# google/deepconsensus

Measured on NVIDIA H100. Metric: zmw_windows_per_sec, higher is better.
Workload: dtype bf16

## Files before the change

deepconsensus_b200/csrc/engine.cu:

```cuda
#include <cuda_bf16.h>
#include <cuda_runtime.h>
#include <math.h>
#include <stdarg.h>
#include <stdio.h>
#include <string.h>

#include <algorithm>
#include <cmath>
#include <functional>
#include <map>
#include <memory>
#include <string>
#include <vector>

#include "../../include/dcb200.h"
#include "../../include/dcb200_debug.h"
#include "kernels.h"

using namespace dcb;

namespace {

thread_local std::string g_create_error;

// ... 556 lines not shown
  epi.x = e->d_x;
  epi.bias = bias;
  if (pos && c.add_pos_encoding) { epi.pe = e->w.pe; epi.pe_img = e->w.pe_img; }
  if (layer < c.num_hidden_layers) {
    epi.xb = e->d_xb;
    if (!c.rezero) { epi.ln_g = e->w.layers[layer].ln_g[sub]; epi.ln_b = e->w.layers[layer].ln_b[sub]; }
  }
  epi.has_xold = has_xold;
  epi.L = e->Lw;
  return epi;
}

struct DbgImage { int stage, which; const DevBuf<__nv_bfloat16>* src; int width; };

std::vector<DbgImage> dbg_images(const dcb_engine* e) {
  const int layers = e->cfg.num_hidden_layers, ff = e->cfg.filter_size;
  std::vector<DbgImage> v = {{0, DCB_DEBUG_EMBED, &e->d_embqkv, e->Epad}, {0, DCB_DEBUG_XB, &e->d_xb, kDP}};
  for (int n = 0; n < layers; ++n) {
    v.insert(v.end(), {{1 + 2 * n, DCB_DEBUG_QKV, &e->d_embqkv, kQKVN}, {1 + 2 * n, DCB_DEBUG_ATT, &e->d_att, kDP},
                       {1 + 2 * n, DCB_DEBUG_XB, &e->d_xb, kDP}, {2 + 2 * n, DCB_DEBUG_HID, &e->d_hid, ff}});
    if (n + 1 < layers) v.push_back({2 + 2 * n, DCB_DEBUG_XB, &e->d_xb, kDP});
  }
  return v;
}

bool dbg_operand_slot(const dcb_engine* e, int stage, int which, size_t* cols, int* width) {
  *cols = 0;
  for (const DbgImage& im : dbg_images(e)) {
    if (im.stage == stage && im.which == which) { *width = im.width; return true; }
    *cols += im.width;
  }
  return false;
}

template <int K, typename T>
int read_capture(dcb_engine* e, const T* image, int iw, int ow, T* out, int64_t out_elems) {
  const int Mlay = e->last_chunk_tokens;
  const int M = Mlay / e->Lw * e->L;
  if (out_elems < (int64_t)M * ow) return fail(e, DCB_ERR_INVALID, "output too small: need %lld", (long long)M * ow);
  CU(e, cudaSetDevice(e->cfg.device));
  std::vector<T> img((size_t)(Mlay + kTileM - 1) / kTileM * kTileM * iw);
  CU(e, cudaMemcpy(img.data(), image, img.size() * sizeof(T), cudaMemcpyDeviceToHost));
  for (int t = 0; t < M; ++t) {
    const int tl = t / e->L * e->Lw + t % e->L;
    const int tile = tl / kTileM, r = tl % kTileM;
    for (int col = 0; col < ow; ++col)
      out[(size_t)t * ow + col] = img[(((size_t)tile * (iw / K) + col / K) * kTileM + r) * K + col % K];
  }
  return DCB_OK;
}

void bf16_forward_chunk(dcb_engine* e, LaunchRecorder& rec, const float* rows_chunk, const uint8_t* packed_chunk,
                        int bw, HeadParams hp, int* d_status) {
  const dcb_config& c = e->cfg;
  const Weights& W = e->w;
  const int L = e->L, Lw = e->Lw, M = bw * Lw;
  const int T = (M + kTileM - 1) / kTileM;
  const cudaStream_t st = rec.st;
  int stage = 0;
  auto snap = [&]() {
    if (e->debug) {
      const size_t ximg = x_image_elems(), cw = (size_t)e->chunk_tiles * kTileM;
      cudaMemcpyAsync(e->d_dbg + (size_t)stage * e->chunk_tiles * ximg, e->d_x, T * ximg * sizeof(float), cudaMemcpyDeviceToDevice, st);
      size_t cols = 0;
      for (const DbgImage& im : dbg_images(e)) {
        if (im.stage == stage)
          cudaMemcpyAsync(e->d_dbg_op + cols * cw, im.src->p, (size_t)T * kTileM * im.width * sizeof(__nv_bfloat16),
                          cudaMemcpyDeviceToDevice, st);
        cols += im.width;
      }
    }
    ++stage;
  };
  rec.run(kProfEmbed, 1, [&] {
    launch_embed(rows_chunk, packed_chunk, e->pl, e->R, L, Lw, M, T, e->echunks, W.cols, W.rowmeta, W.tables,
                 e->table_elems, e->d_embqkv, d_status, st);
  });
  rec.run(kProfRowGemm, 1, [&] {
    launch_gemm_row(e->d_embqkv, W.wc, e->Epad / 16, 2 * (e->Epad / 16), T, row_epi(e, false, nullptr, 0, 0, true), st);
  });
  snap();
  for (int n_ = 0; n_ < c.num_hidden_layers; ++n_) {
    const LayerDev& ld = W.layers[n_];
    rec.run(kProfQkv, 1, [&] { launch_gemm_qkv(e->d_xb, ld.wqkv, T, e->d_embqkv, st); });
    rec.run(kProfAttention, 1, [&] { launch_attention(e->d_embqkv, e->d_att, L, Lw, c.attn_win_size, bw, st); });
    rec.run(kProfRowGemm, 1, [&] {
      launch_gemm_row(e->d_att, ld.wo, kDP / 16, 2 * (kDP / 16), T, row_epi(e, true, nullptr, n_, 1, false), st);
    });
    snap();
    rec.run(kProfFfn, 2, [&] {
      const RowEpi epi = row_epi(e, true, ld.b2, n_ + 1, 0, false);
      __nv_bfloat16* hid = e->debug ? e->d_hid.p : nullptr;
      for (int half = 0; half < 2; ++half) launch_ffn(half, e->d_xb, ld.w1, ld.b1, ld.w2, c.filter_size, T, hid, epi, st);
    });
    if (e->profile) e->prof_ffn_tokens += (long long)bw * L;
    snap();
  }
  hp.x = e->d_x; hp.M = M; hp.L = L; hp.Lw = Lw;
  rec.run(kProfHead, 1, [&] { launch_head(hp, T, st); });
  e->last_chunk_tokens = M;
}

}

extern "C" {

const char* dcb_version(void) { return "dcb200 0.1.0 (sm_90a)"; }

const char* dcb_last_error(const dcb_engine* e) { return e ? e->err.c_str() : g_create_error.c_str(); }

int dcb_create(const dcb_config* cfg, dcb_engine** out) {
  if (!cfg || !out) return fail(nullptr, DCB_ERR_INVALID, "null argument");
  if (cfg->struct_size != (int32_t)sizeof(dcb_config))
    return fail(nullptr, DCB_ERR_INVALID, "dcb_config size mismatch: got %d, built with %zu",
                cfg->struct_size, sizeof(dcb_config));
  if (cfg->hidden_size != kD || cfg->num_heads != kHeads)
    return fail(nullptr, DCB_ERR_INVALID, "unsupported model: hidden_size=%d num_heads=%d (engine is built for %d/%d)",
                cfg->hidden_size, cfg->num_heads, kD, kHeads);
  if (!cfg->condense_transformer_input)
    return fail(nullptr, DCB_ERR_INVALID, "condense_transformer_input must be true");
  if (cfg->filter_size <= 0 || cfg->filter_size % kFFChunk || cfg->filter_size > 2048)
    return fail(nullptr, DCB_ERR_INVALID, "filter_size must be a multiple of %d and <= 2048", kFFChunk);
  if (cfg->max_passes <= 0 || cfg->max_length <= 0 || cfg->max_length > 256 || cfg->num_hidden_layers <= 0 ||
      cfg->max_batch <= 0)
    return fail(nullptr, DCB_ERR_INVALID, "bad max_passes/max_length(<=256)/num_hidden_layers/max_batch");
  if (cfg->precision != DCB_PRECISION_BF16 && cfg->precision != DCB_PRECISION_FP32)
    return fail(nullptr, DCB_ERR_INVALID, "precision must be DCB_PRECISION_BF16 or DCB_PRECISION_FP32");
  int ndev = 0;
  if (cudaGetDeviceCount(&ndev) != cudaSuccess || ndev == 0)
    return fail(nullptr, DCB_ERR_CUDA, "no CUDA device available (the dcb200 engine has no CPU fallback)");
  if (cfg->device < 0 || cfg->device >= ndev) return fail(nullptr, DCB_ERR_INVALID, "bad device ordinal %d", cfg->device);
  cudaDeviceProp prop;
  if (cudaGetDeviceProperties(&prop, cfg->device) != cudaSuccess || prop.major != 9)
    return fail(nullptr, DCB_ERR_CUDA, "device %d is not an sm_90 GPU (compute capability %d.%d)", cfg->device,
                prop.major, prop.minor);

  std::unique_ptr<dcb_engine> eng(new dcb_engine());
  dcb_engine* e = eng.get();
  e->cfg = *cfg;
  e->num_sms = prop.multiProcessorCount;
  e->L = cfg->max_length;
  e->Lw = e->L;
  bool align = true;
#ifdef DCB_DEV_SWITCHES
  if (const char* env = getenv("DCB_ALIGN")) align = atoi(env) != 0;
#endif
  if (align && e->L <= kTileM) e->Lw = kTileM;
  e->R = 4 * cfg->max_passes + (cfg->use_ccs_bq ? 6 : 5);
  e->pl = make_packed_layout(cfg->max_passes, cfg->max_length, cfg->use_ccs_bq ? 1 : 0);
  {
    auto table = [&](const char* layer, int vocab, int width) {
      const int off = (e->table_elems + 7) / 8 * 8;
      e->tables.push_back(EmbedTable{layer, vocab, width, off});
      e->table_elems = off + vocab * width;
      return e->tables.back();
    };
    auto rows = [&](const EmbedTable& tb, int n, float clip, int shift) {
      for (int r = 0; r < n; ++r) {
        e->embed.push_back(StrictEmbedRow{clip, shift, tb.vocab, tb.width, e->E, tb.off});
        e->E += tb.width;
      }
    };
    const int P = cfg->max_passes;
    const EmbedTable bases = table("bases_embedding_layer", kVocab, cfg->per_base_hidden_size);
    rows(bases, P, 0.f, 0);
    rows(table("pw_embedding_layer", cfg->pw_max + 1, cfg->pw_hidden_size), P, (float)cfg->pw_max, 0);
    rows(table("ip_embedding_layer", cfg->ip_max + 1, cfg->ip_hidden_size), P, (float)cfg->ip_max, 0);
    rows(table("strand_embedding_layer", cfg->strand_max + 1, cfg->strand_hidden_size), P, 0.f, 0);
// ... 846 lines not shown
```

deepconsensus_b200/csrc/kernels.cu:

```cuda
#include "kernels.h"

#include <cuda_bf16.h>
#include <math.h>
#include <stdio.h>
#include <stdlib.h>

#include "head_finish.cuh"
#include "sm90.cuh"

namespace dcb {


__global__ void __launch_bounds__(256)
embed_rows_kernel(const float* __restrict__ rows, const uint8_t* __restrict__ packed, PackedLayout pl, int R, int L,
                  int Lw, int M, int echunks,
                  const EmbedCol* __restrict__ cols, const EmbedRow* __restrict__ rowmeta,
                  const __nv_bfloat16* __restrict__ tables, int table_elems,
                  __nv_bfloat16* __restrict__ emb, int* __restrict__ status) {
  extern __shared__ __align__(1024) uint8_t smem[];
  __nv_bfloat16* s_tab = reinterpret_cast<__nv_bfloat16*>(smem);
  const int tab_bytes = (table_elems * 2 + 15) & ~15;
  EmbedCol* s_cols = reinterpret_cast<EmbedCol*>(smem + tab_bytes);
  const int cols_bytes = (echunks * 8 * (int)sizeof(EmbedCol) + 15) & ~15;
  uint16_t* s_ids = reinterpret_cast<uint16_t*>(smem + tab_bytes + cols_bytes);
// ... 477 lines not shown
      wgmma_fence_regs(hacc);
      if (c + 1 == nch) mbar_arrive(a_empty);

      uint32_t af[Cfg::kDownK][4];
      const float* bc = reinterpret_cast<const float*>(stage_base + prev * Cfg::kStageBytes + Cfg::kB1Off) + 2 * q;
#pragma unroll
      for (int kk = 0; kk < Cfg::kDownK; ++kk)
#pragma unroll
        for (int i = 0; i < 4; ++i) {
          const float2 b = *reinterpret_cast<const float2*>(bc + 16 * kk + 8 * (i >> 1));
          af[kk][i] = pack_bf16x2(fmaxf(hacc[8 * kk + 2 * i] + b.x, 0.f), fmaxf(hacc[8 * kk + 2 * i + 1] + b.y, 0.f));
        }
      mbar_arrive(&empty[prev]);
      if constexpr (kHid) {
        __nv_bfloat16* hb = hid + (size_t)tile * kTileM * ff + (size_t)row0 * 8 + 2 * q;
#pragma unroll
        for (int kk = 0; kk < Cfg::kDownK; ++kk)
#pragma unroll
          for (int i = 0; i < 4; ++i)
            *reinterpret_cast<uint32_t*>(hb + ((size_t)(c * 16 + 2 * kk + (i >> 1)) * kTileM + 8 * (i & 1)) * 8) =
                af[kk][i];
      }

#pragma unroll
      for (int kk = 0; kk < Cfg::kDownK; ++kk) {
        mbar_wait(&full[slot], phase);
        const uint32_t st = smem_u32(stage_base + slot * Cfg::kStageBytes);
        wgmma_fence_regs(acc[0]);
        wgmma_fence_regs(acc[1]);
        wgmma_fence();
#pragma unroll
        for (int j = 0; j < 2; ++j)
          wgmma_m64n144k16_rs(acc[j], af[kk], make_kc16_desc(st + j * kNC * 16, kDP * 16, 128), c != 0 || kk != 0);
        wgmma_commit();
        wgmma_fence_regs(acc[0]);
        wgmma_fence_regs(acc[1]);
        wgmma_wait<1>();
        if (kk > 0) {
          wgmma_fence_regs(af[kk - 1]);
          mbar_arrive(&empty[prev]);
        }
        prev = slot;
        next_slot();
      }
      wgmma_wait<0>();
      wgmma_fence_regs(acc[0]);
      wgmma_fence_regs(acc[1]);
      wgmma_fence_regs(af[Cfg::kDownK - 1]);
      mbar_arrive(&empty[prev]);
    }

    row_epilogue<kNC, 2, false>(acc, tile, row0, q, s_vec, epi);
  }
}

constexpr int kAttStride = 144;
constexpr int kAttChunks = kDHP / 8;

__device__ __forceinline__ void mma_bf16_16816(float (&c)[4], const uint32_t (&a)[4], uint32_t b0,
                                               uint32_t b1) {
  asm volatile(
      "mma.sync.aligned.m16n8k16.row.col.f32.bf16.bf16.f32 {%0,%1,%2,%3}, {%4,%5,%6,%7}, {%8,%9}, "
      "{%0,%1,%2,%3};"
      : "+f"(c[0]), "+f"(c[1]), "+f"(c[2]), "+f"(c[3])
      : "r"(a[0]), "r"(a[1]), "r"(a[2]), "r"(a[3]), "r"(b0), "r"(b1));
}

__device__ __forceinline__ void ldmatrix_x2_trans(uint32_t& r0, uint32_t& r1, uint32_t addr) {
  asm volatile("ldmatrix.sync.aligned.m8n8.x2.trans.shared.b16 {%0, %1}, [%2];"
               : "=r"(r0), "=r"(r1)
               : "r"(addr));
}

__device__ __forceinline__ size_t img_off(int tok, int col, int chunks) {
  const int tile = tok / kTileM, r = tok % kTileM;
  return (((size_t)tile * chunks + (col >> 3)) * kTileM + r) * 8 + (col & 7);
}

__device__ __forceinline__ int att_rot(int chunk, int rowmod) {
  const int t = chunk + rowmod;
  return t >= kAttChunks ? t - kAttChunks : t;
}

__global__ void __launch_bounds__(128, 3)
band_attention_kernel(const __nv_bfloat16* __restrict__ qkv, __nv_bfloat16* __restrict__ att,
                      int L, int Lw, int win, int nwindows) {
  extern __shared__ __align__(1024) uint8_t smem[];
  const int w = blockIdx.x >> 1;
  const int head = blockIdx.x & 1;
  if (w >= nwindows) return;
  const int Lp = (L + 15) & ~15;
  __nv_bfloat16* sK = reinterpret_cast<__nv_bfloat16*>(smem);
  __nv_bfloat16* sV = sK + (size_t)Lp * kAttStride;
  constexpr int qkv_chunks = kQKVN / 8;
  const int kcol = (2 + head) * kDHP, vcol = (4 + head) * kDHP, qcol = head * kDHP;
  const int tok0 = w * Lw;

  for (int row = threadIdx.x; row < Lp; row += blockDim.x) {
    const int rm = row % kAttChunks;
    __nv_bfloat16* dk = sK + (size_t)row * kAttStride;
    __nv_bfloat16* dv = sV + (size_t)row * kAttStride;
    if (row < L) {
      const int tok = tok0 + row;
      const size_t base = ((size_t)(tok / kTileM) * qkv_chunks) * kTileM * 8 + (size_t)(tok % kTileM) * 8;
      const __nv_bfloat16* gk = qkv + base + (size_t)(kcol >> 3) * kTileM * 8;
      const __nv_bfloat16* gv = qkv + base + (size_t)(vcol >> 3) * kTileM * 8;
#pragma unroll
      for (int ch = 0; ch < kAttChunks; ++ch) {
        const int pc = att_rot(ch, rm) * 8;
        asm volatile("cp.async.cg.shared.global [%0], [%1], 16;" ::"r"(smem_u32(dk + pc)),
                     "l"(gk + (size_t)ch * kTileM * 8) : "memory");
        asm volatile("cp.async.cg.shared.global [%0], [%1], 16;" ::"r"(smem_u32(dv + pc)),
                     "l"(gv + (size_t)ch * kTileM * 8) : "memory");
      }
    } else {
#pragma unroll
      for (int ch = 0; ch < kAttChunks; ++ch) {
        *reinterpret_cast<uint4*>(dk + ch * 8) = make_uint4(0, 0, 0, 0);
        *reinterpret_cast<uint4*>(dv + ch * 8) = make_uint4(0, 0, 0, 0);
      }
    }
  }
  asm volatile("cp.async.commit_group;" ::: "memory");

  const int warp = threadIdx.x >> 5, lane = threadIdx.x & 31;
  const int g = lane >> 2, t = lane & 3;
  const int band = win > 0 ? win : L;
  constexpr float kLog2e = 1.4426950408889634f;

  constexpr int kChunkElems = kTileM * 8;
  uint32_t qa[kDHP / 16][4];
  auto load_q = [&](int qb) {
    const int r0 = qb * 16 + g, r1 = r0 + 8;
    const __nv_bfloat16* q0 = qkv + img_off(tok0 + (r0 < L ? r0 : 0), qcol + 2 * t, qkv_chunks);
    const __nv_bfloat16* q1 = qkv + img_off(tok0 + (r1 < L ? r1 : 0), qcol + 2 * t, qkv_chunks);
#pragma unroll
    for (int ks = 0; ks < kDHP / 16; ++ks) {
      const uint32_t v0 = __ldg(reinterpret_cast<const uint32_t*>(q0 + (2 * ks) * kChunkElems));
      const uint32_t v1 = __ldg(reinterpret_cast<const uint32_t*>(q1 + (2 * ks) * kChunkElems));
      const uint32_t v2 = __ldg(reinterpret_cast<const uint32_t*>(q0 + (2 * ks + 1) * kChunkElems));
      const uint32_t v3 = __ldg(reinterpret_cast<const uint32_t*>(q1 + (2 * ks + 1) * kChunkElems));
      qa[ks][0] = r0 < L ? v0 : 0u;
      qa[ks][1] = r1 < L ? v1 : 0u;
      qa[ks][2] = r0 < L ? v2 : 0u;
      qa[ks][3] = r1 < L ? v3 : 0u;
    }
  };
  if (warp * 16 < L) load_q(warp);
  asm volatile("cp.async.wait_group 0;" ::: "memory");
  __syncthreads();

  for (int qb = warp; qb * 16 < L; qb += 4) {
    const int i0 = qb * 16;
    const int r0 = i0 + g, r1 = i0 + g + 8;
    if (qb != warp) load_q(qb);
    float o[kDHP / 8][4];
#pragma unroll
    for (int nt = 0; nt < kDHP / 8; ++nt) { o[nt][0] = o[nt][1] = o[nt][2] = o[nt][3] = 0.f; }
    float m0 = -INFINITY, m1 = -INFINITY, l0 = 0.f, l1 = 0.f;

    int jlo = i0 - band; if (jlo < 0) jlo = 0; jlo &= ~15;
    int jhi = i0 + 15 + band + 1; if (jhi > L) jhi = L;
    for (int j0 = jlo; j0 < jhi; j0 += 16) {
      float s[2][4], s2[2][4];
#pragma unroll
      for (int nt = 0; nt < 2; ++nt) {
        s[nt][0] = s[nt][1] = s[nt][2] = s[nt][3] = 0.f;
        s2[nt][0] = s2[nt][1] = s2[nt][2] = s2[nt][3] = 0.f;
      }
      const int krow0 = j0 + g, krow1 = j0 + 8 + g;
      const __nv_bfloat16* kr0 = sK + (size_t)krow0 * kAttStride + 2 * t;
      const __nv_bfloat16* kr1 = sK + (size_t)krow1 * kAttStride + 2 * t;
      const int km0 = krow0 % kAttChunks, km1 = krow1 % kAttChunks;
#pragma unroll
      for (int ks = 0; ks < kDHP / 16; ++ks) {
        const uint32_t a0 = *reinterpret_cast<const uint32_t*>(kr0 + att_rot(2 * ks, km0) * 8);
        const uint32_t a1 = *reinterpret_cast<const uint32_t*>(kr0 + att_rot(2 * ks + 1, km0) * 8);
        const uint32_t c0 = *reinterpret_cast<const uint32_t*>(kr1 + att_rot(2 * ks, km1) * 8);
        const uint32_t c1 = *reinterpret_cast<const uint32_t*>(kr1 + att_rot(2 * ks + 1, km1) * 8);
        if (ks & 1) {
          mma_bf16_16816(s2[0], qa[ks], a0, a1);
          mma_bf16_16816(s2[1], qa[ks], c0, c1);
        } else {
          mma_bf16_16816(s[0], qa[ks], a0, a1);
          mma_bf16_16816(s[1], qa[ks], c0, c1);
        }
      }
#pragma unroll
      for (int nt = 0; nt < 2; ++nt)
#pragma unroll
        for (int e = 0; e < 4; ++e) s[nt][e] += s2[nt][e];
      float tmax0 = -INFINITY, tmax1 = -INFINITY;
#pragma unroll
      for (int nt = 0; nt < 2; ++nt) {
#pragma unroll
        for (int e = 0; e < 4; ++e) {
          const int i = (e < 2) ? r0 : r1;
          const int j = j0 + nt * 8 + 2 * t + (e & 1);
          const int dlt = i - j;
          const bool ok = (j < L) && (dlt <= band) && (dlt >= -band);
          s[nt][e] = ok ? s[nt][e] : -INFINITY;
        }
        tmax0 = fmaxf(tmax0, fmaxf(s[nt][0], s[nt][1]));
        tmax1 = fmaxf(tmax1, fmaxf(s[nt][2], s[nt][3]));
      }
      tmax0 = fmaxf(tmax0, __shfl_xor_sync(0xffffffffu, tmax0, 1));
      tmax0 = fmaxf(tmax0, __shfl_xor_sync(0xffffffffu, tmax0, 2));
      tmax1 = fmaxf(tmax1, __shfl_xor_sync(0xffffffffu, tmax1, 1));
      tmax1 = fmaxf(tmax1, __shfl_xor_sync(0xffffffffu, tmax1, 2));
      const float mn0 = fmaxf(m0, tmax0), mn1 = fmaxf(m1, tmax1);
      const float base0 = mn0 == -INFINITY ? 0.f : mn0, base1 = mn1 == -INFINITY ? 0.f : mn1;
      const float sc0 = exp2f((m0 - base0) * kLog2e), sc1 = exp2f((m1 - base1) * kLog2e);
      m0 = mn0; m1 = mn1;
      float ps0 = 0.f, ps1 = 0.f;
      uint32_t pa[4];
      {
        float p[2][4];
#pragma unroll
        for (int nt = 0; nt < 2; ++nt) {
          p[nt][0] = exp2f((s[nt][0] - base0) * kLog2e);
          p[nt][1] = exp2f((s[nt][1] - base0) * kLog2e);
          p[nt][2] = exp2f((s[nt][2] - base1) * kLog2e);
          p[nt][3] = exp2f((s[nt][3] - base1) * kLog2e);
          ps0 += p[nt][0] + p[nt][1];
          ps1 += p[nt][2] + p[nt][3];
        }
        pa[0] = pack_bf16x2(p[0][0], p[0][1]);
        pa[1] = pack_bf16x2(p[0][2], p[0][3]);
        pa[2] = pack_bf16x2(p[1][0], p[1][1]);
        pa[3] = pack_bf16x2(p[1][2], p[1][3]);
      }
      l0 = l0 * sc0 + ps0;
      l1 = l1 * sc1 + ps1;
      const int vrow = j0 + (lane & 15);
      const int vm = vrow % kAttChunks;
      const uint32_t vbase = smem_u32(sV + (size_t)vrow * kAttStride);
#pragma unroll
      for (int nt = 0; nt < kDHP / 8; ++nt) {
        o[nt][0] *= sc0; o[nt][1] *= sc0; o[nt][2] *= sc1; o[nt][3] *= sc1;
        uint32_t b0, b1;
        ldmatrix_x2_trans(b0, b1, vbase + att_rot(nt, vm) * 16);
        mma_bf16_16816(o[nt], pa, b0, b1);
      }
    }
    l0 += __shfl_xor_sync(0xffffffffu, l0, 1);
    l0 += __shfl_xor_sync(0xffffffffu, l0, 2);
    l1 += __shfl_xor_sync(0xffffffffu, l1, 1);
    l1 += __shfl_xor_sync(0xffffffffu, l1, 2);
    const float inv0 = 1.f / l0, inv1 = 1.f / l1;
    __nv_bfloat16* o0 = att + img_off(tok0 + (r0 < L ? r0 : 0), head * kDHP + 2 * t, kDP / 8);
    __nv_bfloat16* o1 = att + img_off(tok0 + (r1 < L ? r1 : 0), head * kDHP + 2 * t, kDP / 8);
#pragma unroll
    for (int nt = 0; nt < kDHP / 8; ++nt) {
      if (r0 < L)
        *reinterpret_cast<uint32_t*>(o0 + nt * kChunkElems) = pack_bf16x2(o[nt][0] * inv0, o[nt][1] * inv0);
      if (r1 < L)
        *reinterpret_cast<uint32_t*>(o1 + nt * kChunkElems) = pack_bf16x2(o[nt][2] * inv1, o[nt][3] * inv1);
    }
  }
}

__global__ void __launch_bounds__(128)
head_kernel(HeadParams p) {
  __shared__ __align__(16) float sGW[kD * 8];
  __shared__ float sA[kVocab], sBj[kVocab];
  for (int i = threadIdx.x; i < kD * 2; i += blockDim.x)
    reinterpret_cast<float4*>(sGW)[i] = __ldg(reinterpret_cast<const float4*>(p.gw8) + i);
  if (threadIdx.x < kVocab) { sA[threadIdx.x] = p.ab[threadIdx.x]; sBj[threadIdx.x] = p.ab[8 + threadIdx.x]; }
  __syncthreads();
  const int tile = blockIdx.x, r = threadIdx.x;
  const int tok = tile * kTileM + r;
  if (tok >= p.M) return;
  const int wdw = tok / p.Lw, pos = tok - wdw * p.Lw;
  if (pos >= p.L) return;
  const size_t oidx = (size_t)wdw * p.L + pos;
  const float4* xrow = reinterpret_cast<const float4*>(p.x + (size_t)tile * x_image_elems()) + r;
  float s1 = 0.f, s2 = 0.f;
  float t[kVocab];
#pragma unroll
  for (int j = 0; j < kVocab; ++j) t[j] = 0.f;
  const float shift = xrow[0].x;
  constexpr int kHB = 10;
  static_assert((kD / 4) % kHB == 0, "head batch");
#pragma unroll 1
  for (int c0 = 0; c0 < kD / 4; c0 += kHB) {
    float4 v[kHB];
#pragma unroll
    for (int u = 0; u < kHB; ++u) v[u] = xrow[(size_t)(c0 + u) * kTileM];
#pragma unroll
    for (int u = 0; u < kHB; ++u) {
      const float ys[4] = {v[u].x - shift, v[u].y - shift, v[u].z - shift, v[u].w - shift};
#pragma unroll
      for (int i = 0; i < 4; ++i) {
        const int col = (c0 + u) * 4 + i;
        s1 += ys[i];
        s2 = fmaf(ys[i], ys[i], s2);
        const float4 w0 = *reinterpret_cast<const float4*>(&sGW[col * 8]);
        const float w4 = sGW[col * 8 + 4];
        t[0] = fmaf(ys[i], w0.x, t[0]); t[1] = fmaf(ys[i], w0.y, t[1]); t[2] = fmaf(ys[i], w0.z, t[2]);
        t[3] = fmaf(ys[i], w0.w, t[3]); t[4] = fmaf(ys[i], w4, t[4]);
      }
    }
  }
  const float m1 = s1 * (1.f / kD);
  const float rstd = rsqrtf(fmaxf(s2 * (1.f / kD) - m1 * m1, 0.f) + 1e-6f);
  float lg[kVocab];
#pragma unroll
  for (int j = 0; j < kVocab; ++j) lg[j] = rstd * (t[j] - m1 * sA[j]) + sBj[j];
  head_finish(p, lg, oidx);
}

static int g_num_sms = 0;
static int num_sms() {
  if (!g_num_sms) {
    int dev = 0;
    cudaGetDevice(&dev);
    cudaDeviceGetAttribute(&g_num_sms, cudaDevAttrMultiProcessorCount, dev);
    if (g_num_sms <= 0) g_num_sms = 132;
  }
  return g_num_sms;
}


template <int BN, int NCH, int EPI, bool kAres>
static cudaError_t gemm_init() {
  return cudaFuncSetAttribute(gemm_kernel<BN, NCH, EPI, kAres>, cudaFuncAttributeMaxDynamicSharedMemorySize,
                              GemmCfg<BN, NCH, kAres>::kSmemBytes);
}

cudaError_t kernels_init() {
  cudaError_t e;
  if ((e = gemm_init<kNC, 2, EPI_ROW, false>()) != cudaSuccess) return e;
  if ((e = gemm_init<kNC, 1, EPI_QKV, true>()) != cudaSuccess) return e;
  for (auto fn : {ffn_gemm_kernel<false>, ffn_gemm_kernel<true>})
    if ((e = cudaFuncSetAttribute(fn, cudaFuncAttributeMaxDynamicSharedMemorySize, FfnCfg::kSmemBytes)) != cudaSuccess)
      return e;
  e = cudaFuncSetAttribute(embed_rows_kernel, cudaFuncAttributeMaxDynamicSharedMemorySize, 160 * 1024);
  if (e != cudaSuccess) return e;
  e = cudaFuncSetAttribute(band_attention_kernel, cudaFuncAttributeMaxDynamicSharedMemorySize,
                           2 * 256 * kAttStride * 2);
  return e;
}

size_t embed_smem_bytes(int R, int echunks, int table_elems) {
  return (size_t)((table_elems * 2 + 15) & ~15) + ((echunks * 8 * sizeof(EmbedCol) + 15) & ~(size_t)15) +
         (size_t)R * kTileM * 2;
}

void launch_embed(const float* rows, const uint8_t* packed, const PackedLayout& pl, int R, int L, int Lw, int M, int ntiles, int echunks,
                  const EmbedCol* cols, const EmbedRow* rowmeta, const __nv_bfloat16* tables,
                  int table_elems, __nv_bfloat16* emb, int* status, cudaStream_t st) {
  embed_rows_kernel<<<ntiles, 256, embed_smem_bytes(R, echunks, table_elems), st>>>(
      rows, packed, pl, R, L, Lw, M, echunks, cols, rowmeta, tables, table_elems, emb, status);
}

void launch_gemm_row(const __nv_bfloat16* a_img, const __nv_bfloat16* b_img, int a_ksteps, int b_ksteps, int ntiles,
                     const RowEpi& epi, cudaStream_t st) {
  using Cfg = GemmCfg<kNC, 2, false>;
  const int grid = ntiles < num_sms() ? ntiles : num_sms();
  const int smem = Cfg::smem_bytes(Cfg::stages(b_ksteps / Cfg::kSK));
  gemm_kernel<kNC, 2, EPI_ROW, false><<<grid, Cfg::kThreads, smem, st>>>(a_img, b_img, a_ksteps, b_ksteps, ntiles, 1,
                                                                                    nullptr, 0, epi);
}

void launch_gemm_qkv(const __nv_bfloat16* a_img, const __nv_bfloat16* b_img, int ntiles,
                     __nv_bfloat16* qkv_img, cudaStream_t st) {
  using Cfg = GemmCfg<kNC, 1, true>;
  const int npairs = (ntiles + 1) / 2;
  const int grid = npairs < num_sms() ? npairs : num_sms();
  RowEpi none{};
  gemm_kernel<kNC, 1, EPI_QKV, true><<<grid, Cfg::kThreads, Cfg::kSmemBytes, st>>>(
      a_img, b_img, kDP / 16, 2 * (kDP / 16), ntiles, kQKVN / kQKVGroup, qkv_img, kQKVN / 8, none);
}

void launch_ffn(int half, const __nv_bfloat16* xb_img, const __nv_bfloat16* w1_img, const float* b1,
                const __nv_bfloat16* w2_img, int ff, int ntiles, __nv_bfloat16* hid_img, const RowEpi& epi,
                cudaStream_t st) {
  const int split = (ntiles + 1) / 2;
  const int t0 = half ? split : 0, t1 = half ? ntiles : split;
  const int n = t1 - t0;
  const int grid = n < 1 ? 1 : n < num_sms() ? n : num_sms();
  if (hid_img)
    ffn_gemm_kernel<true><<<grid, FfnCfg::kThreads, FfnCfg::kSmemBytes, st>>>(xb_img, w1_img, b1, w2_img, ff, t0, t1,
                                                                              hid_img, epi);
  else
    ffn_gemm_kernel<false><<<grid, FfnCfg::kThreads, FfnCfg::kSmemBytes, st>>>(xb_img, w1_img, b1, w2_img, ff, t0, t1,
                                                                               nullptr, epi);
}

__global__ void __launch_bounds__(256)
unpack_rows_kernel(const uint8_t* __restrict__ packed, PackedLayout pl, int nwindows, float* __restrict__ rows) {
  const int b = blockIdx.x;
  const uint8_t* w = packed + (size_t)b * pl.stride;
  float* out = rows + (size_t)b * pl.R * pl.L;
  for (int i = threadIdx.x; i < pl.R * pl.L; i += blockDim.x) {
    const int r = i / pl.L, l = i - r * pl.L;
    out[i] = packed_value(pl, w, r, l);
  }
}

void launch_unpack_rows(const uint8_t* packed, const PackedLayout& pl, int nwindows, float* rows, cudaStream_t st) {
  if (nwindows > 0) unpack_rows_kernel<<<nwindows, 256, 0, st>>>(packed, pl, nwindows, rows);
}


void launch_attention(const __nv_bfloat16* qkv, __nv_bfloat16* att, int L, int Lw, int win, int nwindows,
                      cudaStream_t st) {
  const int Lp = (L + 15) & ~15;
  const size_t smem = (size_t)2 * Lp * kAttStride * 2;
  band_attention_kernel<<<nwindows * 2, 128, smem, st>>>(qkv, att, L, Lw, win, nwindows);
}



__global__ void __launch_bounds__(256)
stitch_kernel(const uint8_t* __restrict__ bases, const uint8_t* __restrict__ quals, int L,
              const int32_t* __restrict__ zmw_start, uint8_t* __restrict__ seq_out, uint8_t* __restrict__ qual_out,
              int32_t* __restrict__ len_out) {
  __shared__ int s_warp[8];
  __shared__ int s_total;
  const int z = blockIdx.x;
  const size_t off = (size_t)zmw_start[z] * L;
  const int n = (zmw_start[z + 1] - zmw_start[z]) * L;
  const uint8_t* in_b = bases + off;
  const uint8_t* in_q = quals + off;
  uint8_t* out_b = seq_out + off;
  uint8_t* out_q = qual_out + off;
  const int warp = threadIdx.x >> 5, lane = threadIdx.x & 31;
  int running = 0;
  for (int t0 = 0; t0 < n; t0 += 1024) {
    uint8_t b[4], q[4];
    int cnt = 0;
#pragma unroll
    for (int k = 0; k < 4; ++k) {
      const int idx = t0 + threadIdx.x * 4 + k;
      b[k] = idx < n ? in_b[idx] : (uint8_t)' ';
      q[k] = idx < n ? in_q[idx] : (uint8_t)0;
      cnt += b[k] != (uint8_t)' ';
    }
    int incl = cnt;
#pragma unroll
    for (int d = 1; d < 32; d <<= 1) {
      const int v = __shfl_up_sync(0xffffffffu, incl, d);
      if (lane >= d) incl += v;
    }
    if (lane == 31) s_warp[warp] = incl;
    __syncthreads();
    if (threadIdx.x == 0) {
      int acc = 0;
      for (int w = 0; w < 8; ++w) { const int v = s_warp[w]; s_warp[w] = acc; acc += v; }
      s_total = acc;
    }
    __syncthreads();
    int pos = running + s_warp[warp] + incl - cnt;
#pragma unroll
    for (int k = 0; k < 4; ++k) {
      if (b[k] != (uint8_t)' ') {
        out_b[pos] = b[k];
        out_q[pos] = q[k];
        ++pos;
      }
    }
    running += s_total;
    __syncthreads();
  }
  if (threadIdx.x == 0) len_out[z] = running;
}

void launch_stitch(const uint8_t* bases, const uint8_t* quals, int L, const int32_t* zmw_start, int n_zmw,
                   uint8_t* seq_out, uint8_t* qual_out, int32_t* len_out, cudaStream_t st) {
  if (n_zmw > 0) stitch_kernel<<<n_zmw, 256, 0, st>>>(bases, quals, L, zmw_start, seq_out, qual_out, len_out);
}

void launch_head(const HeadParams& p, int ntiles, cudaStream_t st) {
  head_kernel<<<ntiles, 128, 0, st>>>(p);
}

}
```

deepconsensus_b200/csrc/kernels.h:

```cpp
#pragma once
#include <cuda_runtime.h>

#include "common.h"

namespace dcb {

cudaError_t kernels_init();

size_t embed_smem_bytes(int R, int echunks, int table_elems);
void launch_embed(const float* rows, const uint8_t* packed, const PackedLayout& pl, int R, int L, int Lw, int M, int ntiles, int echunks,
                  const EmbedCol* cols, const EmbedRow* rowmeta, const __nv_bfloat16* tables,
                  int table_elems, __nv_bfloat16* emb, int* status, cudaStream_t st);
void launch_gemm_row(const __nv_bfloat16* a_img, const __nv_bfloat16* b_img, int a_ksteps, int b_ksteps, int ntiles,
                     const RowEpi& epi, cudaStream_t st);
void launch_gemm_qkv(const __nv_bfloat16* a_img, const __nv_bfloat16* b_img, int ntiles,
                     __nv_bfloat16* qkv_img, cudaStream_t st);
void launch_ffn(int half, const __nv_bfloat16* xb_img, const __nv_bfloat16* w1_img, const float* b1,
                const __nv_bfloat16* w2_img, int ff, int ntiles, __nv_bfloat16* hid_img, const RowEpi& epi,
                cudaStream_t st);
void launch_unpack_rows(const uint8_t* packed, const PackedLayout& pl, int nwindows, float* rows, cudaStream_t st);
void launch_attention(const __nv_bfloat16* qkv, __nv_bfloat16* att, int L, int Lw, int win, int nwindows,
                      cudaStream_t st);
void launch_head(const HeadParams& p, int ntiles, cudaStream_t st);
void launch_stitch(const uint8_t* bases, const uint8_t* quals, int L, const int32_t* zmw_start, int n_zmw,
                   uint8_t* seq_out, uint8_t* qual_out, int32_t* len_out, cudaStream_t st);


void launch_read_outcome(const uint8_t* qual, const int32_t* len, const int32_t* zmw_start, const int32_t* window_pos,
                         int L, int n_zmw, const double* p10, double min_quality, int min_length, int32_t* outcome,
                         double* avg_q, cudaStream_t st);
void launch_fastq(const uint8_t* seq, const uint8_t* qual, const int32_t* len, const int32_t* zmw_start, int L, int n_zmw,
                  const int32_t* outcome, const uint8_t* names, const int32_t* name_off, int64_t* rec_off, uint8_t* fastq,
                  int64_t cap, cudaStream_t st);
void launch_skip_mask(const int16_t* ccs_bq, int n_windows, int L, const double* p10, double thr, uint8_t* mask,
                      double* avg_out, cudaStream_t st);
void launch_fill_skipped(const uint8_t* ccs_ids, const int16_t* ccs_bq, const int32_t* dst, int k, int L, int calib_enabled,
                         double thr, double cw, double cb, int max_q, uint8_t* bases, uint8_t* quals, int* status,
                         cudaStream_t st);
void launch_head_epilogue(const float* logits, int n, const HeadParams& p, cudaStream_t st);

constexpr int kReadMeta = 10;
struct PrepZmw {
  int32_t read0, n_reads;
  int32_t keep;
  int32_t ccs_off, ccs_len, bq_any;
  int32_t mb;
  int32_t wb;
  int32_t win_off, win_cap;
  int64_t gap_off;
  int64_t plane_off;
};
struct PrepBatch {
  int n_zmw, ins_trim;
  PackedLayout pl;
  const PrepZmw* zmw;
  const int32_t* read_meta;
  const float* read_sn;
  const uint32_t* cigar;
  const uint8_t *bases, *pw, *ip, *ccs_bases, *ccs_bq;
  int4* op_scan;
  int32_t* read_noni_qs;
  int32_t* gap;
  uint8_t* spaced;
  int2* win_list;
  int4* zmw_out;
  int* status;
};
struct PrepWindows {
  int32_t* zmw_windows;
  int2* window;
  int32_t* window_pos;
  uint8_t* overflow;
  int32_t* num_passes;
  uint8_t* ccs_ids;
  int16_t* ccs_bq;
};
void launch_prep_layout(const PrepBatch& b, const PrepWindows& out, cudaStream_t st);
void launch_prep_pack(const PrepBatch& b, const int2* window, const int32_t* list, int n_list, int n_windows, uint8_t* packed,
                      cudaStream_t st);

cudaError_t launch_evaluate(const float* probs, const uint8_t* labels, const uint8_t* ccs_ids, int B, int L,
                            float del_cost, float loss_reg, int hard_min, float* loss, uint8_t* exact,
                            int32_t* pred_counts, int32_t* ccs_counts, cudaStream_t st);
cudaError_t loss_grad_grid(int B, int* ctas);
size_t loss_grad_table_bytes(int L, int ctas);
cudaError_t launch_loss_grad(const float* probs, const uint8_t* labels, int B, int L, float del_cost, float loss_reg,
                             int hard_min, float* tables, int ctas, float* loss, float* grad, float* matches,
                             cudaStream_t st);
cudaError_t launch_distill_loss_grad(const float* teacher, const float* student, int B, int L, float temperature,
                                     int logit_loss, float* loss, float* grad, cudaStream_t st);

void launch_strict_embed(const float* rows, int R, int L, int E, int nwindows, const StrictEmbedRow* meta,
                         const float* tables, float* emb, int* status, cudaStream_t st);
void launch_strict_gemm(const float* A, const float* B, float* C, int M, int N, int K, const StrictEpi& ep,
                        cudaStream_t st);
void launch_strict_layernorm(const float* x, float* y, int M, const float* g, const float* b, cudaStream_t st);
void launch_strict_attention(const float* q, const float* k, const float* v, float* o, int nwindows, int L, int win,
                             cudaStream_t st);
void launch_strict_head(const float* x, int M, const HeadParams& hp, cudaStream_t st);

}
```

Baseline: 148,300.

## Fuse QKV projection GEMM with band attention in a warp-specialized kernel

When each window fits exactly one M-tile, a new kernel computes Q, K and V per head with wgmma, writes K and V straight into shared memory, keeps Q in registers, and runs the band attention in the same block. A producer warp streams weight stages through mbarriers. This removes the global round trip of the QKV activations and one kernel launch per layer. The attention inner loop is factored into a shared device function. The costs are one block per SM with heavy shared memory, weights re-streamed for every tile, and serialization between the GEMM and attention phases inside a block.

```diff
diff --git a/deepconsensus_b200/csrc/engine.cu b/deepconsensus_b200/csrc/engine.cu
--- a/deepconsensus_b200/csrc/engine.cu
+++ b/deepconsensus_b200/csrc/engine.cu
@@ -662,8 +662,16 @@
   snap();
   for (int n_ = 0; n_ < c.num_hidden_layers; ++n_) {
     const LayerDev& ld = W.layers[n_];
-    rec.run(kProfQkv, 1, [&] { launch_gemm_qkv(e->d_xb, ld.wqkv, T, e->d_embqkv, st); });
-    rec.run(kProfAttention, 1, [&] { launch_attention(e->d_embqkv, e->d_att, L, Lw, c.attn_win_size, bw, st); });
+    if (Lw == kTileM) {
+      rec.run(kProfAttention, 2, [&] {
+        __nv_bfloat16* qkv = e->debug ? e->d_embqkv.p : nullptr;
+        for (int half = 0; half < 2; ++half)
+          launch_qkv_attention(half, e->d_xb, ld.wqkv, L, c.attn_win_size, T, qkv, e->d_att, st);
+      });
+    } else {
+      rec.run(kProfQkv, 1, [&] { launch_gemm_qkv(e->d_xb, ld.wqkv, T, e->d_embqkv, st); });
+      rec.run(kProfAttention, 1, [&] { launch_attention(e->d_embqkv, e->d_att, L, Lw, c.attn_win_size, bw, st); });
+    }
     rec.run(kProfRowGemm, 1, [&] {
       launch_gemm_row(e->d_att, ld.wo, kDP / 16, 2 * (kDP / 16), T, row_epi(e, true, nullptr, n_, 1, false), st);
     });
diff --git a/deepconsensus_b200/csrc/kernels.cu b/deepconsensus_b200/csrc/kernels.cu
--- a/deepconsensus_b200/csrc/kernels.cu
+++ b/deepconsensus_b200/csrc/kernels.cu
@@ -583,6 +583,119 @@
   return t >= kAttChunks ? t - kAttChunks : t;
 }
 
+__device__ __forceinline__ void attend_block(const uint32_t (&qa)[kDHP / 16][4], const __nv_bfloat16* sK,
+                                             const __nv_bfloat16* sV, int i0, int L, int band,
+                                             __nv_bfloat16* __restrict__ att, int tok0, int head) {
+  const int lane = threadIdx.x & 31;
+  const int g = lane >> 2, t = lane & 3;
+  constexpr float kLog2e = 1.4426950408889634f;
+  constexpr int kChunkElems = kTileM * 8;
+  const int r0 = i0 + g, r1 = i0 + g + 8;
+  float o[kDHP / 8][4];
+#pragma unroll
+  for (int nt = 0; nt < kDHP / 8; ++nt) { o[nt][0] = o[nt][1] = o[nt][2] = o[nt][3] = 0.f; }
+  float m0 = -INFINITY, m1 = -INFINITY, l0 = 0.f, l1 = 0.f;
+
+  int jlo = i0 - band; if (jlo < 0) jlo = 0; jlo &= ~15;
+  int jhi = i0 + 15 + band + 1; if (jhi > L) jhi = L;
+  for (int j0 = jlo; j0 < jhi; j0 += 16) {
+    float s[2][4], s2[2][4];
+#pragma unroll
+    for (int nt = 0; nt < 2; ++nt) {
+      s[nt][0] = s[nt][1] = s[nt][2] = s[nt][3] = 0.f;
+      s2[nt][0] = s2[nt][1] = s2[nt][2] = s2[nt][3] = 0.f;
+    }
+    const int krow0 = j0 + g, krow1 = j0 + 8 + g;
+    const __nv_bfloat16* kr0 = sK + (size_t)krow0 * kAttStride + 2 * t;
+    const __nv_bfloat16* kr1 = sK + (size_t)krow1 * kAttStride + 2 * t;
+    const int km0 = krow0 % kAttChunks, km1 = krow1 % kAttChunks;
+#pragma unroll
+    for (int ks = 0; ks < kDHP / 16; ++ks) {
+      const uint32_t a0 = *reinterpret_cast<const uint32_t*>(kr0 + att_rot(2 * ks, km0) * 8);
+      const uint32_t a1 = *reinterpret_cast<const uint32_t*>(kr0 + att_rot(2 * ks + 1, km0) * 8);
+      const uint32_t c0 = *reinterpret_cast<const uint32_t*>(kr1 + att_rot(2 * ks, km1) * 8);
+      const uint32_t c1 = *reinterpret_cast<const uint32_t*>(kr1 + att_rot(2 * ks + 1, km1) * 8);
+      if (ks & 1) {
+        mma_bf16_16816(s2[0], qa[ks], a0, a1);
+        mma_bf16_16816(s2[1], qa[ks], c0, c1);
+      } else {
+        mma_bf16_16816(s[0], qa[ks], a0, a1);
+        mma_bf16_16816(s[1], qa[ks], c0, c1);
+      }
+    }
+#pragma unroll
+    for (int nt = 0; nt < 2; ++nt)
+#pragma unroll
+      for (int e = 0; e < 4; ++e) s[nt][e] += s2[nt][e];
+    float tmax0 = -INFINITY, tmax1 = -INFINITY;
+#pragma unroll
+    for (int nt = 0; nt < 2; ++nt) {
+#pragma unroll
+      for (int e = 0; e < 4; ++e) {
+        const int i = (e < 2) ? r0 : r1;
+        const int j = j0 + nt * 8 + 2 * t + (e & 1);
+        const int dlt = i - j;
+        const bool ok = (j < L) && (dlt <= band) && (dlt >= -band);
+        s[nt][e] = ok ? s[nt][e] : -INFINITY;
+      }
+      tmax0 = fmaxf(tmax0, fmaxf(s[nt][0], s[nt][1]));
+      tmax1 = fmaxf(tmax1, fmaxf(s[nt][2], s[nt][3]));
+    }
+    tmax0 = fmaxf(tmax0, __shfl_xor_sync(0xffffffffu, tmax0, 1));
+    tmax0 = fmaxf(tmax0, __shfl_xor_sync(0xffffffffu, tmax0, 2));
+    tmax1 = fmaxf(tmax1, __shfl_xor_sync(0xffffffffu, tmax1, 1));
+    tmax1 = fmaxf(tmax1, __shfl_xor_sync(0xffffffffu, tmax1, 2));
+    const float mn0 = fmaxf(m0, tmax0), mn1 = fmaxf(m1, tmax1);
+    const float base0 = mn0 == -INFINITY ? 0.f : mn0, base1 = mn1 == -INFINITY ? 0.f : mn1;
+    const float sc0 = exp2f((m0 - base0) * kLog2e), sc1 = exp2f((m1 - base1) * kLog2e);
+    m0 = mn0; m1 = mn1;
+    float ps0 = 0.f, ps1 = 0.f;
+    uint32_t pa[4];
+    {
+      float p[2][4];
+#pragma unroll
+      for (int nt = 0; nt < 2; ++nt) {
+        p[nt][0] = exp2f((s[nt][0] - base0) * kLog2e);
+        p[nt][1] = exp2f((s[nt][1] - base0) * kLog2e);
+        p[nt][2] = exp2f((s[nt][2] - base1) * kLog2e);
+        p[nt][3] = exp2f((s[nt][3] - base1) * kLog2e);
+        ps0 += p[nt][0] + p[nt][1];
+        ps1 += p[nt][2] + p[nt][3];
+      }
+      pa[0] = pack_bf16x2(p[0][0], p[0][1]);
+      pa[1] = pack_bf16x2(p[0][2], p[0][3]);
+      pa[2] = pack_bf16x2(p[1][0], p[1][1]);
+      pa[3] = pack_bf16x2(p[1][2], p[1][3]);
+    }
+    l0 = l0 * sc0 + ps0;
+    l1 = l1 * sc1 + ps1;
+    const int vrow = j0 + (lane & 15);
+    const int vm = vrow % kAttChunks;
+    const uint32_t vbase = smem_u32(sV + (size_t)vrow * kAttStride);
+#pragma unroll
+    for (int nt = 0; nt < kDHP / 8; ++nt) {
+      o[nt][0] *= sc0; o[nt][1] *= sc0; o[nt][2] *= sc1; o[nt][3] *= sc1;
+      uint32_t b0, b1;
+      ldmatrix_x2_trans(b0, b1, vbase + att_rot(nt, vm) * 16);
+      mma_bf16_16816(o[nt], pa, b0, b1);
+    }
+  }
+  l0 += __shfl_xor_sync(0xffffffffu, l0, 1);
+  l0 += __shfl_xor_sync(0xffffffffu, l0, 2);
+  l1 += __shfl_xor_sync(0xffffffffu, l1, 1);
+  l1 += __shfl_xor_sync(0xffffffffu, l1, 2);
+  const float inv0 = 1.f / l0, inv1 = 1.f / l1;
+  __nv_bfloat16* o0 = att + img_off(tok0 + (r0 < L ? r0 : 0), head * kDHP + 2 * t, kDP / 8);
+  __nv_bfloat16* o1 = att + img_off(tok0 + (r1 < L ? r1 : 0), head * kDHP + 2 * t, kDP / 8);
+#pragma unroll
+  for (int nt = 0; nt < kDHP / 8; ++nt) {
+    if (r0 < L)
+      *reinterpret_cast<uint32_t*>(o0 + nt * kChunkElems) = pack_bf16x2(o[nt][0] * inv0, o[nt][1] * inv0);
+    if (r1 < L)
+      *reinterpret_cast<uint32_t*>(o1 + nt * kChunkElems) = pack_bf16x2(o[nt][2] * inv1, o[nt][3] * inv1);
+  }
+}
+
 __global__ void __launch_bounds__(128, 3)
 band_attention_kernel(const __nv_bfloat16* __restrict__ qkv, __nv_bfloat16* __restrict__ att,
                       int L, int Lw, int win, int nwindows) {
@@ -627,7 +740,6 @@
   const int warp = threadIdx.x >> 5, lane = threadIdx.x & 31;
   const int g = lane >> 2, t = lane & 3;
   const int band = win > 0 ? win : L;
-  constexpr float kLog2e = 1.4426950408889634f;
 
   constexpr int kChunkElems = kTileM * 8;
   uint32_t qa[kDHP / 16][4];
@@ -652,111 +764,170 @@
   __syncthreads();
 
   for (int qb = warp; qb * 16 < L; qb += 4) {
-    const int i0 = qb * 16;
-    const int r0 = i0 + g, r1 = i0 + g + 8;
     if (qb != warp) load_q(qb);
-    float o[kDHP / 8][4];
-#pragma unroll
-    for (int nt = 0; nt < kDHP / 8; ++nt) { o[nt][0] = o[nt][1] = o[nt][2] = o[nt][3] = 0.f; }
-    float m0 = -INFINITY, m1 = -INFINITY, l0 = 0.f, l1 = 0.f;
-
-    int jlo = i0 - band; if (jlo < 0) jlo = 0; jlo &= ~15;
-    int jhi = i0 + 15 + band + 1; if (jhi > L) jhi = L;
-    for (int j0 = jlo; j0 < jhi; j0 += 16) {
-      float s[2][4], s2[2][4];
-#pragma unroll
-      for (int nt = 0; nt < 2; ++nt) {
-        s[nt][0] = s[nt][1] = s[nt][2] = s[nt][3] = 0.f;
-        s2[nt][0] = s2[nt][1] = s2[nt][2] = s2[nt][3] = 0.f;
-      }
-      const int krow0 = j0 + g, krow1 = j0 + 8 + g;
-      const __nv_bfloat16* kr0 = sK + (size_t)krow0 * kAttStride + 2 * t;
-      const __nv_bfloat16* kr1 = sK + (size_t)krow1 * kAttStride + 2 * t;
-      const int km0 = krow0 % kAttChunks, km1 = krow1 % kAttChunks;
-#pragma unroll
-      for (int ks = 0; ks < kDHP / 16; ++ks) {
-        const uint32_t a0 = *reinterpret_cast<const uint32_t*>(kr0 + att_rot(2 * ks, km0) * 8);
-        const uint32_t a1 = *reinterpret_cast<const uint32_t*>(kr0 + att_rot(2 * ks + 1, km0) * 8);
-        const uint32_t c0 = *reinterpret_cast<const uint32_t*>(kr1 + att_rot(2 * ks, km1) * 8);
-        const uint32_t c1 = *reinterpret_cast<const uint32_t*>(kr1 + att_rot(2 * ks + 1, km1) * 8);
-        if (ks & 1) {
-          mma_bf16_16816(s2[0], qa[ks], a0, a1);
-          mma_bf16_16816(s2[1], qa[ks], c0, c1);
+    attend_block(qa, sK, sV, qb * 16, L, band, att, tok0, head);
+  }
+}
+
+struct QkvAttCfg {
+  static constexpr int kAK = kDP / 16;
+  static constexpr int kSK = 2;
+  static constexpr int kGroupStages = 2 * kAK / kSK;
+  static constexpr int kABytesPerK = 2 * kTileM * 16;
+  static constexpr int kBBytesPerK = 2 * kQKVGroup * 16;
+  static constexpr int kStageBytes = kSK * kBBytesPerK;
+  static constexpr int kGroupBytes = 2 * kAK * kBBytesPerK;
+  static constexpr int kStages = 8;
+  static constexpr int kATileBytes = kAK * kABytesPerK;
+  static constexpr int kKVBytes = kTileM * kAttStride * 2;
+  static constexpr int kBarBytes = 256;
+  static constexpr int kSmemBytes = kATileBytes + 2 * kKVBytes + kStages * kStageBytes + kBarBytes;
+  static constexpr int kThreads = 384;
+  static_assert(kSmemBytes <= 232448, "over the sm_90 opt-in shared memory per block");
+  static_assert((2 * kStages + 2) * 8 <= kBarBytes, "the mbarriers (full, empty, a_full, a_empty) fit");
+  static_assert(kQKVGroup == kDHP && kQKVN == 6 * kQKVGroup, "one n-group is one head's q, k or v");
+};
+
+__device__ __forceinline__ int qkv_att_group(int i) {
+  const int h = i / 3, part = i % 3;
+  return part == 0 ? 2 + h : part == 1 ? 4 + h : h;
+}
+
+__device__ __forceinline__ void consumer_bar_sync() { asm volatile("bar.sync 1, 256;" ::: "memory"); }
+
+template <bool kQkv>
+__global__ void __launch_bounds__(384, 1)
+qkv_attention_kernel(const __nv_bfloat16* __restrict__ xb_img, const __nv_bfloat16* __restrict__ b_img, int L,
+                     int win, int tile_begin, int tile_end, __nv_bfloat16* __restrict__ qkv_img,
+                     __nv_bfloat16* __restrict__ att) {
+  using Cfg = QkvAttCfg;
+  extern __shared__ __align__(1024) uint8_t smem[];
+  uint8_t* a_res = smem;
+  __nv_bfloat16* sK = reinterpret_cast<__nv_bfloat16*>(smem + Cfg::kATileBytes);
+  __nv_bfloat16* sV = reinterpret_cast<__nv_bfloat16*>(smem + Cfg::kATileBytes + Cfg::kKVBytes);
+  uint8_t* stage_base = smem + Cfg::kATileBytes + 2 * Cfg::kKVBytes;
+  uint64_t* full = reinterpret_cast<uint64_t*>(stage_base + Cfg::kStages * Cfg::kStageBytes);
+  uint64_t* empty = full + Cfg::kStages;
+  uint64_t* a_full = empty + Cfg::kStages;
+  uint64_t* a_empty = a_full + 1;
+
+  const int warp = threadIdx.x >> 5;
+  const int lane = threadIdx.x & 31;
+  if (threadIdx.x == 0) {
+    for (int i = 0; i < Cfg::kStages; ++i) {
+      mbar_init(&full[i], 1);
+      mbar_init(&empty[i], 256);
+    }
+    mbar_init(a_full, 1);
+    mbar_init(a_empty, 256);
+    mbar_fence_init();
+  }
+  __syncthreads();
+
+  if (warp >= 8) {
+    setmaxnreg_dec<24>();
+    if (warp == 8 && lane == 0) {
+      uint32_t slot = 0, phase = 0, it = 0;
+      for (int tile = tile_begin + blockIdx.x; tile < tile_end; tile += gridDim.x, ++it) {
+        mbar_wait(a_empty, (it & 1) ^ 1);
+        mbar_arrive_expect_tx(a_full, Cfg::kATileBytes);
+        bulk_g2s(a_res, reinterpret_cast<const uint8_t*>(xb_img) + (size_t)tile * Cfg::kATileBytes, Cfg::kATileBytes,
+                 a_full);
+        for (int i = 0; i < 6; ++i) {
+          const uint8_t* b_src = reinterpret_cast<const uint8_t*>(b_img) + (size_t)qkv_att_group(i) * Cfg::kGroupBytes;
+          for (int s = 0; s < Cfg::kGroupStages; ++s) {
+            mbar_wait(&empty[slot], phase ^ 1);
+            mbar_arrive_expect_tx(&full[slot], Cfg::kStageBytes);
+            bulk_g2s(stage_base + slot * Cfg::kStageBytes, b_src + (size_t)s * Cfg::kStageBytes, Cfg::kStageBytes,
+                     &full[slot]);
+            if (++slot == Cfg::kStages) { slot = 0; phase ^= 1; }
+          }
+        }
+      }
+    }
+    return;
+  }
+
+  setmaxnreg_inc<240>();
+  const int wg = warp >> 2;
+  const int g = lane >> 2, q = lane & 3;
+  const int row0 = wg * 64 + (warp & 3) * 16 + g;
+  const uint32_t a_base = smem_u32(a_res) + wg * 64 * 16;
+  const int band = win > 0 ? win : L;
+  float acc[kQKVGroup / 2];
+  uint32_t slot = 0, phase = 0, it = 0;
+  for (int tile = tile_begin + blockIdx.x; tile < tile_end; tile += gridDim.x, ++it) {
+    mbar_wait(a_full, it & 1);
+#pragma unroll 1
+    for (int h = 0; h < kHeads; ++h) {
+      uint32_t qa[kDHP / 16][4];
+#pragma unroll
+      for (int part = 0; part < 3; ++part) {
+        uint32_t prev = 0;
+#pragma unroll 1
+        for (int s = 0; s < Cfg::kGroupStages; ++s) {
+          mbar_wait(&full[slot], phase);
+          const uint32_t st = smem_u32(stage_base + slot * Cfg::kStageBytes);
+          wgmma_fence_regs(acc);
+          wgmma_fence();
+#pragma unroll
+          for (int kk = 0; kk < Cfg::kSK; ++kk) {
+            const uint64_t adesc =
+                make_kc16_desc(a_base + ((s * Cfg::kSK + kk) % Cfg::kAK) * Cfg::kABytesPerK, kTileM * 16, 128);
+            const uint64_t bdesc = make_kc16_desc(st + kk * Cfg::kBBytesPerK, kQKVGroup * 16, 128);
+            wgmma_m64n144k16(acc, adesc, bdesc, (s | kk) != 0);
+          }
+          wgmma_commit();
+          wgmma_fence_regs(acc);
+          wgmma_wait<1>();
+          if (s > 0) mbar_arrive(&empty[prev]);
+          prev = slot;
+          if (++slot == Cfg::kStages) { slot = 0; phase ^= 1; }
+        }
+        wgmma_wait<0>();
+        wgmma_fence_regs(acc);
+        mbar_arrive(&empty[prev]);
+        if (h + 1 == kHeads && part == 2) mbar_arrive(a_empty);
+
+        const int grp = part == 0 ? 2 + h : part == 1 ? 4 + h : h;
+        if constexpr (kQkv) {
+          __nv_bfloat16* obase = qkv_img + (size_t)tile * kTileM * (kQKVN / 8) * 8;
+#pragma unroll
+          for (int hr = 0; hr < 2; ++hr)
+#pragma unroll
+            for (int jj = 0; jj < kQKVGroup / 8; ++jj) {
+              const int col = grp * kQKVGroup + jj * 8 + 2 * q;
+              *reinterpret_cast<uint32_t*>(obase + ((size_t)(col >> 3) * kTileM + row0 + 8 * hr) * 8 + (col & 7)) =
+                  pack_bf16x2(acc[jj * 4 + 2 * hr], acc[jj * 4 + 2 * hr + 1]);
+            }
+        }
+        if (part < 2) {
+          if (part == 0) consumer_bar_sync();
+          __nv_bfloat16* dst = part == 0 ? sK : sV;
+#pragma unroll
+          for (int hr = 0; hr < 2; ++hr) {
+            const int r = row0 + 8 * hr;
+            const int rm = r % kAttChunks;
+            __nv_bfloat16* drow = dst + (size_t)r * kAttStride + 2 * q;
+#pragma unroll
+            for (int jj = 0; jj < kDHP / 8; ++jj)
+              *reinterpret_cast<uint32_t*>(drow + att_rot(jj, rm) * 8) =
+                  r < L ? pack_bf16x2(acc[jj * 4 + 2 * hr], acc[jj * 4 + 2 * hr + 1]) : 0u;
+          }
         } else {
-          mma_bf16_16816(s[0], qa[ks], a0, a1);
-          mma_bf16_16816(s[1], qa[ks], c0, c1);
-        }
-      }
-#pragma unroll
-      for (int nt = 0; nt < 2; ++nt)
-#pragma unroll
-        for (int e = 0; e < 4; ++e) s[nt][e] += s2[nt][e];
-      float tmax0 = -INFINITY, tmax1 = -INFINITY;
-#pragma unroll
-      for (int nt = 0; nt < 2; ++nt) {
-#pragma unroll
-        for (int e = 0; e < 4; ++e) {
-          const int i = (e < 2) ? r0 : r1;
-          const int j = j0 + nt * 8 + 2 * t + (e & 1);
-          const int dlt = i - j;
-          const bool ok = (j < L) && (dlt <= band) && (dlt >= -band);
-          s[nt][e] = ok ? s[nt][e] : -INFINITY;
-        }
-        tmax0 = fmaxf(tmax0, fmaxf(s[nt][0], s[nt][1]));
-        tmax1 = fmaxf(tmax1, fmaxf(s[nt][2], s[nt][3]));
-      }
-      tmax0 = fmaxf(tmax0, __shfl_xor_sync(0xffffffffu, tmax0, 1));
-      tmax0 = fmaxf(tmax0, __shfl_xor_sync(0xffffffffu, tmax0, 2));
-      tmax1 = fmaxf(tmax1, __shfl_xor_sync(0xffffffffu, tmax1, 1));
-      tmax1 = fmaxf(tmax1, __shfl_xor_sync(0xffffffffu, tmax1, 2));
-      const float mn0 = fmaxf(m0, tmax0), mn1 = fmaxf(m1, tmax1);
-      const float base0 = mn0 == -INFINITY ? 0.f : mn0, base1 = mn1 == -INFINITY ? 0.f : mn1;
-      const float sc0 = exp2f((m0 - base0) * kLog2e), sc1 = exp2f((m1 - base1) * kLog2e);
-      m0 = mn0; m1 = mn1;
-      float ps0 = 0.f, ps1 = 0.f;
-      uint32_t pa[4];
-      {
-        float p[2][4];
-#pragma unroll
-        for (int nt = 0; nt < 2; ++nt) {
-          p[nt][0] = exp2f((s[nt][0] - base0) * kLog2e);
-          p[nt][1] = exp2f((s[nt][1] - base0) * kLog2e);
-          p[nt][2] = exp2f((s[nt][2] - base1) * kLog2e);
-          p[nt][3] = exp2f((s[nt][3] - base1) * kLog2e);
-          ps0 += p[nt][0] + p[nt][1];
-          ps1 += p[nt][2] + p[nt][3];
-        }
-        pa[0] = pack_bf16x2(p[0][0], p[0][1]);
-        pa[1] = pack_bf16x2(p[0][2], p[0][3]);
-        pa[2] = pack_bf16x2(p[1][0], p[1][1]);
-        pa[3] = pack_bf16x2(p[1][2], p[1][3]);
-      }
-      l0 = l0 * sc0 + ps0;
-      l1 = l1 * sc1 + ps1;
-      const int vrow = j0 + (lane & 15);
-      const int vm = vrow % kAttChunks;
-      const uint32_t vbase = smem_u32(sV + (size_t)vrow * kAttStride);
-#pragma unroll
-      for (int nt = 0; nt < kDHP / 8; ++nt) {
-        o[nt][0] *= sc0; o[nt][1] *= sc0; o[nt][2] *= sc1; o[nt][3] *= sc1;
-        uint32_t b0, b1;
-        ldmatrix_x2_trans(b0, b1, vbase + att_rot(nt, vm) * 16);
-        mma_bf16_16816(o[nt], pa, b0, b1);
-      }
-    }
-    l0 += __shfl_xor_sync(0xffffffffu, l0, 1);
-    l0 += __shfl_xor_sync(0xffffffffu, l0, 2);
-    l1 += __shfl_xor_sync(0xffffffffu, l1, 1);
-    l1 += __shfl_xor_sync(0xffffffffu, l1, 2);
-    const float inv0 = 1.f / l0, inv1 = 1.f / l1;
-    __nv_bfloat16* o0 = att + img_off(tok0 + (r0 < L ? r0 : 0), head * kDHP + 2 * t, kDP / 8);
-    __nv_bfloat16* o1 = att + img_off(tok0 + (r1 < L ? r1 : 0), head * kDHP + 2 * t, kDP / 8);
-#pragma unroll
-    for (int nt = 0; nt < kDHP / 8; ++nt) {
-      if (r0 < L)
-        *reinterpret_cast<uint32_t*>(o0 + nt * kChunkElems) = pack_bf16x2(o[nt][0] * inv0, o[nt][1] * inv0);
-      if (r1 < L)
-        *reinterpret_cast<uint32_t*>(o1 + nt * kChunkElems) = pack_bf16x2(o[nt][2] * inv1, o[nt][3] * inv1);
+          const bool v0 = row0 < L, v1 = row0 + 8 < L;
+#pragma unroll
+          for (int ks = 0; ks < kDHP / 16; ++ks) {
+            qa[ks][0] = v0 ? pack_bf16x2(acc[8 * ks + 0], acc[8 * ks + 1]) : 0u;
+            qa[ks][1] = v1 ? pack_bf16x2(acc[8 * ks + 2], acc[8 * ks + 3]) : 0u;
+            qa[ks][2] = v0 ? pack_bf16x2(acc[8 * ks + 4], acc[8 * ks + 5]) : 0u;
+            qa[ks][3] = v1 ? pack_bf16x2(acc[8 * ks + 6], acc[8 * ks + 7]) : 0u;
+          }
+        }
+      }
+      consumer_bar_sync();
+      const int i0 = warp * 16;
+      if (i0 < L) attend_block(qa, sK, sV, i0, L, band, att, tile * kTileM, h);
     }
   }
 }
@@ -836,6 +1007,10 @@
   for (auto fn : {ffn_gemm_kernel<false>, ffn_gemm_kernel<true>})
     if ((e = cudaFuncSetAttribute(fn, cudaFuncAttributeMaxDynamicSharedMemorySize, FfnCfg::kSmemBytes)) != cudaSuccess)
       return e;
+  for (auto fn : {qkv_attention_kernel<false>, qkv_attention_kernel<true>})
+    if ((e = cudaFuncSetAttribute(fn, cudaFuncAttributeMaxDynamicSharedMemorySize, QkvAttCfg::kSmemBytes)) !=
+        cudaSuccess)
+      return e;
   e = cudaFuncSetAttribute(embed_rows_kernel, cudaFuncAttributeMaxDynamicSharedMemorySize, 160 * 1024);
   if (e != cudaSuccess) return e;
   e = cudaFuncSetAttribute(band_attention_kernel, cudaFuncAttributeMaxDynamicSharedMemorySize,
@@ -910,6 +1085,20 @@
   const int Lp = (L + 15) & ~15;
   const size_t smem = (size_t)2 * Lp * kAttStride * 2;
   band_attention_kernel<<<nwindows * 2, 128, smem, st>>>(qkv, att, L, Lw, win, nwindows);
+}
+
+void launch_qkv_attention(int half, const __nv_bfloat16* xb_img, const __nv_bfloat16* wqkv, int L, int win,
+                          int ntiles, __nv_bfloat16* qkv_img, __nv_bfloat16* att, cudaStream_t st) {
+  const int split = (ntiles + 1) / 2;
+  const int t0 = half ? split : 0, t1 = half ? ntiles : split;
+  const int n = t1 - t0;
+  const int grid = n < 1 ? 1 : n < num_sms() ? n : num_sms();
+  if (qkv_img)
+    qkv_attention_kernel<true><<<grid, QkvAttCfg::kThreads, QkvAttCfg::kSmemBytes, st>>>(xb_img, wqkv, L, win, t0, t1,
+                                                                                        qkv_img, att);
+  else
+    qkv_attention_kernel<false><<<grid, QkvAttCfg::kThreads, QkvAttCfg::kSmemBytes, st>>>(xb_img, wqkv, L, win, t0,
+                                                                                         t1, nullptr, att);
 }
 
 
diff --git a/deepconsensus_b200/csrc/kernels.h b/deepconsensus_b200/csrc/kernels.h
--- a/deepconsensus_b200/csrc/kernels.h
+++ b/deepconsensus_b200/csrc/kernels.h
@@ -21,6 +21,8 @@
 void launch_unpack_rows(const uint8_t* packed, const PackedLayout& pl, int nwindows, float* rows, cudaStream_t st);
 void launch_attention(const __nv_bfloat16* qkv, __nv_bfloat16* att, int L, int Lw, int win, int nwindows,
                       cudaStream_t st);
+void launch_qkv_attention(int half, const __nv_bfloat16* xb_img, const __nv_bfloat16* wqkv, int L, int win,
+                          int ntiles, __nv_bfloat16* qkv_img, __nv_bfloat16* att, cudaStream_t st);
 void launch_head(const HeadParams& p, int ntiles, cudaStream_t st);
 void launch_stitch(const uint8_t* bases, const uint8_t* quals, int L, const int32_t* zmw_start, int n_zmw,
                    uint8_t* seq_out, uint8_t* qual_out, int32_t* len_out, cudaStream_t st);
```

Measured after the change: 160,200, median of 6. 8.1% higher.
